# emiliofidalgo/liodom

Measured on AMD Instinct MI355X. Metric: scans/sec (64×1800 cloud, prev_frames=20) at 1 GPU; pose RMSE vs CPU ref, higher is better.
Workload: dtype f64

## Files before the change

### liodom_amd/csrc/handle_plan.h

```cpp
#pragma once
#include <algorithm>
#include <climits>
#include <cstdio>
#include <cstdlib>
#include <cstring>

#include "../../include/liodom_hip.h"
#include "liodom_sizes.h"

namespace liodom_dev {

struct HandleEnv {
  bool pipe_flags = true;
  bool map_rows = true;
  int hash_build = -1;
  int lds_cells_max = kLdsCellsMax;
  bool early_rebuild = true;
  bool safe_mode = false;
  int debug_clocks = 0;
  bool ring_split = true;
  bool ring_split_lb = true;
  int ring_pitch = 0;
  bool hash_incr = true;
  float rebuild_delta = 0.25f;
// ... 219 lines not shown
  const long long ring_pitch = env.ring_pitch ? env.ring_pitch : round_up(cdiv((long long)config->max_points * 9, (long long)H * 8), 8);

  if (ts > (1LL << 30) || map_cap > INT_MAX || used_cap > INT_MAX || sorted_cap > INT_MAX || ring_id_stride > INT_MAX || ring_pitch > INT_MAX) {
    *error = "liodom_create: capacities (window, received map, points per scan) exceed 32-bit sizes";
    return LIODOM_ERR_CAPACITY;
  }
  p.map_cap = (int)map_cap; p.table_size = (int)ts;
  p.used_cap = (int)used_cap; p.ovf_base = (int)ovf_base; p.sorted_cap = (int)sorted_cap;
  p.ring_id_stride = (size_t)ring_id_stride;
  p.ring_pitch = (int)ring_pitch;
  p.ring_stride = p.ring_split_lb ? std::max((size_t)config->max_points, (size_t)H * (size_t)p.ring_pitch) : (size_t)config->max_points;

  p.ring_split = env.ring_split && !p.safe_mode;
  if (p.ring_split) {
    long long budget = (long long)std::max(0, caps.ring_split_wgs_per_cu) * std::max(0, caps.cus) / 2;
    if (budget > 256) budget = 256;
    p.ring_split_max_wgs = (int)budget;
    if (p.tile_cap > p.ring_split_max_wgs) p.ring_split = false;
  }

  p.knn8 = p.lockstep && env.knn8;
  p.knn8_grid = (int)std::max(1LL, cdiv(cdiv(p.edge_cap, kKnn8Queries), kKnnGridDiv));
  p.hash_incr = (env.hash_incr && p.knn8 && p.lds_hash_build && !params->mapping && !params->filter_local_map && P > kHbPeriod &&
                 sorted_cap >= 2 * map_cap + (long long)(kHbPeriod - 1) * p.edge_cap) ? 1 : 0;
  p.hb_spill_base = p.sorted_cap - (kHbPeriod - 1) * p.edge_cap;
  p.knn_queries = p.lockstep ? 4 : 8;
  p.knn_partials = p.lockstep ? 0 : 1;
  p.knn_blocks = (int)round_up(cdiv(p.edge_cap, p.knn_queries), 4);
  p.knn_grid = (int)std::max(1LL, cdiv(p.knn_blocks, kKnnGridDiv));
  p.mask_stride = (int)round_up(p.knn_blocks, 128);

  p.ov_ok = env.knn_overlap != 0 && p.early_rebuild && S == 1 && p.knn_partials &&
            (env.knn_overlap == 2 || (long long)p.knn_grid * 4 * 3 <= (long long)caps.cus * 24);
  p.chain_ok = p.early_rebuild && S == 1 && p.knn_partials && !p.use_imu && (long long)p.knn_grid * 4 * 2 <= (long long)caps.cus * 24 &&
               env.knn_overlap != 0 && env.chain;
  p.speculate = (p.ov_ok || p.chain_ok) ? env.speculate : 0;
  p.spec_backoff = 16;
  p.spec_theta = env.spec_theta;

  *out = p;
  return LIODOM_OK;
}

struct OverlapModes { bool ov, chain; };
inline OverlapModes plan_overlap_modes(const HandlePlan& p, bool alone) {
  const bool base = p.early_rebuild && p.use_flags && alone;
  return {base && p.ov_ok, base && p.chain_ok && !p.flag_gate};
}

struct ModesRuntime {
  bool alone = true;
  bool streams_concurrent = true;
  int hb_stats[4] = {0, 0, 0, 0}, spec_stats[4] = {0, 0, 0, 0};
  unsigned int chain_count = 0, done0 = 0, done1 = 0;
  double replay_enqueue_us = 0.0, replay_wait_us = 0.0;
  int n_lagged = 0, n_readers = 0, n_hits = 0;
  long long subset_steps = 0;
};

inline void plan_format_modes(const HandlePlan& p, const ModesRuntime& r, char* buf, int cap) {
  const OverlapModes om = plan_overlap_modes(p, r.alone);
  snprintf(buf, (size_t)cap,
           "n_streams=%d early_rebuild=%d hash_build=%s pipe_flags=%d flag_gate=%d lm_groups=%d knn_instance=%d knn_queries=%d "
           "knn_grid=%d/%d knn8=%d hash_incr=%d hash_rebuilds=%d hash_appends=%d hash_appends_spilled=%d hash_points_spilled=%d knn_partials=%d knn_saved_bound=%d knn_exact_only=%d line_gate_kernel=%d filter_local_map=%d mapping=%d "
           "rotation_mode=%d table_size=%d sorted_cap=%d hb_spill_base=%d rebuild_delta=%.3f knn_overlap=%d streams_concurrent=%d safe_mode=%d ring_split=%d ring_split_max_wgs=%d ring_split_lb=%d chain=%d speculate=%d spec_early=%d/%d spec_unconfirmed=%d/%d chain_done=%u/%u/%u replay_enqueue_us=%.2f replay_wait_us=%.2f debug=%d",
           p.n_streams, p.early_rebuild, p.early_rebuild ? "streamed" : (p.lds_hash_build ? "lds" : "global"), p.use_flags ? 1 : 0,
           (p.use_flags && p.flag_gate) ? 1 : 0, p.lm_groups, p.lockstep ? 128 : 256, p.knn_queries, p.knn_grid,
           p.knn_blocks, p.knn8 ? 1 : 0, p.hash_incr, r.hb_stats[0], r.hb_stats[1], r.hb_stats[2], r.hb_stats[3], p.knn_partials,
           p.knn_save >= 2 ? 2 : (p.knn_save >= 1 ? 1 : 0), p.knn_exact_only, p.lockstep ? 1 : 0, p.filter_local_map, p.mapping,
           p.rotation_mode, p.table_size, p.sorted_cap, p.hb_spill_base, (double)p.rebuild_delta,
           (om.ov || om.chain) ? 1 : 0, r.streams_concurrent ? 1 : 0, p.safe_mode ? 1 : 0, p.ring_split ? 1 : 0, p.ring_split ? p.ring_split_max_wgs : 0, p.ring_split_lb ? 1 : 0,
           om.chain ? 1 : 0, p.speculate, r.spec_stats[0], r.spec_stats[2], r.spec_stats[1], r.spec_stats[3], r.chain_count, r.done0, r.done1,
           r.replay_enqueue_us, r.replay_wait_us, p.debug);
  auto tail = [&](size_t* room) { const size_t n = std::strlen(buf); *room = (size_t)cap - n; return buf + n; };
  size_t room = 0;
  if (p.pose_covariance) { char* t = tail(&room); snprintf(t, room, " pose_cov=1"); }
  if (r.n_lagged > 0) { char* t = tail(&room); snprintf(t, room, " mapper_lag=%d", r.n_lagged); }
  if (r.n_readers > 0) { char* t = tail(&room); snprintf(t, room, " map_readers=%d map_rows=%d", r.n_readers, p.map_rows ? 1 : 0); }
  if (r.n_hits > 0) { char* t = tail(&room); snprintf(t, room, " map_hits=%d", r.n_hits); }
  { char* t = tail(&room); snprintf(t, room, " subset_steps=%lld", r.subset_steps); }
}

}
```

### liodom_amd/csrc/kernels_knn.h

```cpp
constexpr float kCellInv = 1.0f;
constexpr double kCellSize = 1.0;

struct Top5 {
  unsigned long long k0, k1, k2, k3, k4;
  int p0, p1, p2, p3, p4;
};
constexpr unsigned long long kTop5Empty = (0x7f800000ull << 32) | 0x7fffffffull;
__device__ __forceinline__ float top5_dist(unsigned long long k) { return __int_as_float((int)(k >> 32)); }
__device__ __forceinline__ int top5_index(unsigned long long k) { return (int)(unsigned int)(k & 0xFFFFFFFFull); }
#define TOP5_STAGE(K, P)                                          \
  {                                                               \
    const bool lt = ck < (K);                                     \
    const unsigned long long nk = lt ? ck : (K);                  \
    const int np = lt ? cp : (P);                                 \
    ck = lt ? (K) : ck;                                           \
    cp = lt ? (P) : cp;                                           \
    (K) = nk; (P) = np;                                           \
  }
__device__ __forceinline__ void top5_insert(Top5& t, float d, int wi, int pos) {
  unsigned long long ck = ((unsigned long long)(unsigned int)__float_as_int(d) << 32) | (unsigned int)wi;
  int cp = pos;
  if (ck < t.k4) {
    TOP5_STAGE(t.k0, t.p0)
    TOP5_STAGE(t.k1, t.p1)
// ... 169 lines not shown


__device__ __forceinline__ void knn_merge(Top5& t, Top5& g, int hl, int half_shift) {
  unsigned long long gk[5]; int gp[5];
#pragma unroll
  for (int r = 0; r < 5; r++) {
    const unsigned long long key = t.k0;
    const unsigned int dmin = half_min_u32((unsigned int)(key >> 32));
    unsigned int win = (unsigned int)((__ballot((unsigned int)(key >> 32) == dmin) >> half_shift) & 0xFFFFFFFFull);
    unsigned long long mk;
    if (__popc(win) == 1) {
      mk = ((unsigned long long)dmin << 32) | (unsigned int)__shfl((int)(unsigned int)(key & 0xFFFFFFFFull), __ffs(win) - 1, kKnnGroup);
    } else {
      mk = half_min_u64(key);
      win = (unsigned int)((__ballot(key == mk) >> half_shift) & 0xFFFFFFFFull);
    }
    const int wl = __ffs(win) - 1;
    gp[r] = __shfl(t.p0, wl, kKnnGroup);
    gk[r] = mk;
    if (hl == wl) {
      t.k0 = t.k1; t.k1 = t.k2; t.k2 = t.k3; t.k3 = t.k4; t.k4 = kTop5Empty;
      t.p0 = t.p1; t.p1 = t.p2; t.p2 = t.p3; t.p3 = t.p4; t.p4 = -1;
    }
  }
  g.k0 = gk[0]; g.k1 = gk[1]; g.k2 = gk[2]; g.k3 = gk[3]; g.k4 = gk[4];
  g.p0 = gp[0]; g.p1 = gp[1]; g.p2 = gp[2]; g.p3 = gp[3]; g.p4 = gp[4];
}

__device__ void rebuild_alloc(const DevView& v, int s, StreamState& st, int block, int nblocks);
__device__ void rebuild_count_and_pad(const DevView& v, int s, StreamState& st, int eb, int block, int* sbase, int* sslot, bool keep);

template <int kQ>
struct KnnShared {
  int incl[kQ][kKnnGroup];
  int adj[kQ][kKnnGroup];
  float nn[kQ][16];
  int res[kQ][4];
  double part[kQ][32];
  double blk[kQ][24];
};

__device__ __forceinline__ float best2_bound(const Best2Acc& t, int half_shift) {
  float B = 1.0f;
  const float thr[4] = {0.36f, 0.09f, 0.0225f, 0.0036f};
#pragma unroll
  for (int k = 0; k < 4; k++) {
    const int c = __popc((unsigned int)(__ballot(t.m1 <= thr[k]) >> half_shift)) + __popc((unsigned int)(__ballot(t.m2 <= thr[k]) >> half_shift));
    B = c >= 5 ? thr[k] : B;
  }
  return B;
}

template <class Tune>
__device__ __forceinline__ void knn_probe_cells(const DevView& v, const StreamState& st, int fc, int hl, int cx, int cy, int cz, float qx, float qy, float qz,
                                                const CellSlot* cells, const unsigned int* bits, unsigned int tmask,
                                                unsigned int& start, unsigned int& cnt, float& lb) {
  if (hl < 27) {
    const int dx = hl % 3 - 1, dy = (hl / 3) % 3 - 1, dz = hl / 9 - 1;
    const unsigned long long key = pack_cell(cx + dx, cy + dy, cz + dz);
    unsigned int h = hash_cell(key, tmask);
    if (Tune::kProbeBoth) {
      const unsigned int word = bits[h >> 5];
      const uint4 raw = *reinterpret_cast<const uint4*>(cells + h);
      const unsigned long long k = ((unsigned long long)raw.y << 32) | raw.x;
      bool more = ((word >> (h & 31)) & 1u) != 0u;
      if (more && k == key) { start = raw.z; cnt = raw.w; more = false; }
      for (int pr = 1; more && pr < v.table_size; pr++) {
        h = (h + 1) & tmask;
        if (!((bits[h >> 5] >> (h & 31)) & 1u)) break;
        const uint4 r2 = *reinterpret_cast<const uint4*>(cells + h);
        if ((((unsigned long long)r2.y << 32) | r2.x) == key) { start = r2.z; cnt = r2.w; break; }
      }
    } else {
      for (int pr = 0; pr < v.table_size; pr++) {
        if (!((bits[h >> 5] >> (h & 31)) & 1u)) break;
        const uint4 raw = *reinterpret_cast<const uint4*>(cells + h);
        const unsigned long long k = ((unsigned long long)raw.y << 32) | raw.x;
        if (k == key) { start = raw.z; cnt = raw.w; break; }
        h = (h + 1) & tmask;
      }
    }
    const float cs = (float)kCellSize;
    const float lx = (float)(cx + dx) * cs, ly = (float)(cy + dy) * cs, lz = (float)(cz + dz) * cs;
    const float ex = qx < lx ? lx - qx : (qx > lx + cs ? qx - (lx + cs) : 0.0f);
    const float ey = qy < ly ? ly - qy : (qy > ly + cs ? qy - (ly + cs) : 0.0f);
    const float ez = qz < lz ? lz - qz : (qz > lz + cs ? qz - (lz + cs) : 0.0f);
    lb = (ex * ex + ey * ey + ez * ez) * (1.0f - 1e-5f);
  } else if (hl == 27 && v.early_rebuild) {
    start = (unsigned int)v.ovf_base;
    cnt = (unsigned int)st.n_ovf[LD_TAB_PARITY(v, fc)];
  }
}

struct KnnPre {
  float gsq;
  float4 sq;
  int p[5];
  float4 c[5];
};
constexpr float kOvMargin = 0.03f;
#ifndef LIODOM_OV_MARGIN_PER_M
#define LIODOM_OV_MARGIN_PER_M 0.004f
#endif
constexpr float kOvMarginPerMetre = LIODOM_OV_MARGIN_PER_M;
constexpr float kOvMarginMax = 0.30f;
template <int kKnnThreads>
__device__ __forceinline__ void knn_presearch(const DevView& v, int s, const StreamState& st, int fc, int e, int E,
                                              KnnShared<kKnnThreads / kKnnGroup>& sh, KnnPre& pre, float range) {
  typedef KnnTune<(kKnnThreads >= 256)> Tune;
  const int grp = threadIdx.x / kKnnGroup, hl = threadIdx.x & (kKnnGroup - 1);
  const int ec = e < v.edge_cap ? e : v.edge_cap - 1;
  pre.gsq = 0.f;
  pre.sq = make_float4(0.f, 0.f, 0.f, __int_as_float(0x7f800000));
#pragma unroll
  for (int k = 0; k < 5; k++) { pre.p[k] = -1; pre.c[k] = make_float4(0.f, 0.f, 0.f, 0.f); }
  if (!v.knn_save_q) return;
  pre.sq = v.knn_save_q[(size_t)s * v.edge_cap + ec];
  const float qx = pre.sq.x, qy = pre.sq.y, qz = pre.sq.z;
  const bool act = e < E && !v.knn_exact_only && ld_isfinite((double)qx) && ld_isfinite((double)qy) && ld_isfinite((double)qz) &&
                   fabsf(qx) < 1.0e9f && fabsf(qy) < 1.0e9f && fabsf(qz) < 1.0e9f;
  if (!act) return;
  const int cx = (int)floorf(qx * kCellInv), cy = (int)floorf(qy * kCellInv), cz = (int)floorf(qz * kCellInv);
  const unsigned int tmask = st.table_mask;
  const int stab = s + LD_TAB_PARITY(v, fc) * v.n_streams;
  const CellSlot* cells = v.cells + (size_t)stab * v.table_size;
  const unsigned int* bits = v.cell_bits + (size_t)stab * (v.table_size >> 5);
  const float4* sp = v.sorted_pts + (size_t)stab * v.sorted_cap;
  unsigned int start = 0, cnt = 0;
  float lb = 0.0f;
  knn_probe_cells<Tune>(v, st, fc, hl, cx, cy, cz, qx, qy, qz, cells, bits, tmask, start, cnt, lb);
  const float margin = fminf(kOvMargin + kOvMarginPerMetre * range, kOvMarginMax);
  const float r = fminf(sqrtf(pre.sq.w), 1.0f) + margin;
  const float B = r * r * (1.0f + 1e-5f);
  Top5Acc ta;
  {
    const unsigned long long sentinel = ((unsigned long long)(unsigned int)__float_as_int(B) << 32) | 0x7fffffffull;
    ta.t.k0 = ta.t.k1 = ta.t.k2 = ta.t.k3 = ta.t.k4 = sentinel;
    ta.t.p0 = ta.t.p1 = ta.t.p2 = ta.t.p3 = ta.t.p4 = -1;
  }
  const bool all = cnt > 0 && !(lb > B);
  knn_stream_cells<Top5Acc, 2, 2, 64>(ta, sp, sh.incl[grp], sh.adj[grp], start, all ? cnt : 0u, hl, qx, qy, qz);
  float gl = B;
  if (ta.t.p4 >= 0) gl = fminf(gl, top5_dist(ta.t.k4));
  pre.gsq = __int_as_float((int)half_min_u32((unsigned int)__float_as_int(gl)));
  pre.p[0] = ta.t.p0; pre.p[1] = ta.t.p1; pre.p[2] = ta.t.p2; pre.p[3] = ta.t.p3; pre.p[4] = ta.t.p4;
#pragma unroll
  for (int k = 0; k < 5; k++) pre.c[k] = sp[pre.p[k] >= 0 ? pre.p[k] : 0];
}

template <int kKnnThreads, bool kPre = false, bool kTail = true, bool kWt = kPre>
__device__ __forceinline__ void knn_block(const DevView& v, int s, StreamState& st, int fc, int outer_it, int eb, int bv, int E,
                                          KnnShared<kKnnThreads / kKnnGroup>& sh, const float4& p_in, const double (&T_in)[12],
                                          const KnnPre& pre, const double* qt) {
  constexpr int kKnnQueries = kKnnThreads / kKnnGroup;
  typedef KnnTune<(kKnnThreads >= 256)> Tune;
  const int grp = threadIdx.x / kKnnGroup;
  const int e = bv * kKnnQueries + grp;
  const int hl = threadIdx.x & (kKnnGroup - 1);
  const int half_shift = (threadIdx.x & 32);
  const bool dbgb = (bv == 5) && (s == 0) && (threadIdx.x == 0) && (outer_it == 0);
  const unsigned long long t_blk = (kInstrument && (v.debug & 32)) ? wall_clock64() : 0ull;
  DBG_STAMP(v, dbgb, 1, 0);
  bool active = e < E;
  float qx = 0.f, qy = 0.f, qz = 0.f;
  if (active) {
    float4 p = p_in;
    double T[12];
#pragma unroll
    for (int i = 0; i < 12; i++) T[i] = T_in[i];
    if (!Tune::kHoistLoads) {
      p = v.edges[((size_t)eb * v.n_streams + s) * v.edge_cap + e];
#pragma unroll
      for (int i = 0; i < 12; i++) T[i] = st.odom[i];
    }
    transform_point(T, p.x, p.y, p.z, &qx, &qy, &qz);
    if (v.knn_q && hl == 0) v.knn_q[((size_t)s * 2 + outer_it) * v.edge_cap + e] = make_float4(qx, qy, qz, 0.f);
    active = ld_isfinite((double)qx) && ld_isfinite((double)qy) && ld_isfinite((double)qz) &&
             fabsf(qx) < 1.0e9f && fabsf(qy) < 1.0e9f && fabsf(qz) < 1.0e9f;
  }
  DBG_STAMP(v, dbgb, 1, 1); DBG_QSTAMP(1);
  if (hl == 0) { sh.res[grp][0] = 0; sh.res[grp][1] = -1; sh.res[grp][2] = -1; }
  float d5 = __int_as_float(0x7f800000);
  if (active) {
    const int cx = (int)floorf(qx * kCellInv), cy = (int)floorf(qy * kCellInv), cz = (int)floorf(qz * kCellInv);
    const unsigned int tmask = st.table_mask;
    const int stab = s + LD_TAB_PARITY(v, fc) * v.n_streams;
    const CellSlot* cells = v.cells + (size_t)stab * v.table_size;
    const unsigned int* bits = v.cell_bits + (size_t)stab * (v.table_size >> 5);
    const float4* sp = v.sorted_pts + (size_t)stab * v.sorted_cap;
    float d5_r = __int_as_float(0x7f800000);
    int pos5[5] = {-1, -1, -1, -1, -1};
    bool reranked = false;
    if (kPre) {
      if ((kInstrument && (v.debug & 64)) && hl == 0 && !(pre.gsq > 0.f)) atomicAdd(&v.dbg_clk[262], 1ull);
      if (pre.gsq > 0.f) {
        Top5 t, g;
        top5_clear(t);
#pragma unroll
        for (int k = 0; k < 5; k++) {
          if (pre.p[k] >= 0) top5_insert(t, sqdist_f(qx, qy, qz, pre.c[k].x, pre.c[k].y, pre.c[k].z), __float_as_int(pre.c[k].w), pre.p[k]);
        }
        knn_merge(t, g, hl, half_shift);
        const float d5n = g.p4 >= 0 ? top5_dist(g.k4) : __int_as_float(0x7f800000);
        const double ddx = (double)qx - (double)pre.sq.x, ddy = (double)qy - (double)pre.sq.y, ddz = (double)qz - (double)pre.sq.z;
        const double delta = sqrt(ddx * ddx + ddy * ddy + ddz * ddz) * (1.0 + 1e-12);
        const double r = sqrt((double)pre.gsq) * (1.0 - 2e-7) - delta;
        double limit = r > 0.0 ? r * r * (1.0 - 1e-6) : 0.0;
        {
          const double cs = kCellSize;
          const double fx = (double)qx - (double)(int)floorf(pre.sq.x * kCellInv) * cs, fy = (double)qy - (double)(int)floorf(pre.sq.y * kCellInv) * cs,
                       fz = (double)qz - (double)(int)floorf(pre.sq.z * kCellInv) * cs;
          const double edge = fmin(fmin(fmin(fx, cs - fx), fmin(fy, cs - fy)), fmin(fz, cs - fz));
          const double ro = (cs + edge) * (1.0 - 2e-7);
          const double lo = ro > 0.0 ? ro * ro * (1.0 - 1e-6) : 0.0;
          limit = limit < lo ? limit : lo;
        }
        reranked = (double)d5n < limit || limit > 1.0;
        if ((kInstrument && (v.debug & 64)) && hl == 0) {
          atomicAdd(&v.dbg_clk[261], 1ull);
          if (!reranked) {
            const float rn = fminf(sqrtf(pre.sq.w), 1.0f) + kOvMargin;
            atomicAdd(&v.dbg_clk[g.p4 < 0 ? 264 : 265], 1ull);
            if (delta > 0.01) atomicAdd(&v.dbg_clk[266], 1ull);
            if (pre.gsq < rn * rn) atomicAdd(&v.dbg_clk[267], 1ull);
            if (!(pre.sq.w < 1.0f)) atomicAdd(&v.dbg_clk[268], 1ull);
            if (delta > 0.03) atomicAdd(&v.dbg_clk[269], 1ull);
          }
        }
        if (reranked) {
          d5_r = d5n;
          pos5[0] = g.p0; pos5[1] = g.p1; pos5[2] = g.p2; pos5[3] = g.p3; pos5[4] = g.p4;
          if (d5n < 1.0f) {
#pragma unroll
            for (int k = 0; k < 5; k++) {
              if (pre.p[k] >= 0) {
                const int r = pre.p[k] == g.p0 ? 0 : pre.p[k] == g.p1 ? 1 : pre.p[k] == g.p2 ? 2 : pre.p[k] == g.p3 ? 3 : pre.p[k] == g.p4 ? 4 : -1;
                if (r >= 0) {
                  sh.nn[grp][r * 3 + 0] = pre.c[k].x; sh.nn[grp][r * 3 + 1] = pre.c[k].y; sh.nn[grp][r * 3 + 2] = pre.c[k].z;
                  if (r < 2) sh.res[grp][1 + r] = __float_as_int(pre.c[k].w);
                }
              }
            }
            if (hl == 0) sh.res[grp][0] = 1;
          }
        }
      }
    } else
    if (outer_it == 1 && v.knn_save_pos && !v.knn_exact_only) {
      const float gsq = v.knn_save_g[(size_t)s * v.edge_cap + e];
      if (gsq > 0.f) {
        const float4 sq = v.knn_save_q[(size_t)s * v.edge_cap + e];
        const int2 sv = v.knn_save_pos[((size_t)s * v.edge_cap + e) * kKnnGroup + hl];
        const float4 m0 = sp[sv.x >= 0 ? sv.x : 0], m1 = sp[sv.y >= 0 ? sv.y : 0];
        Best2Acc br;
        br.clear();
        br.consider(sv.x >= 0, sqdist_f(qx, qy, qz, m0.x, m0.y, m0.z), 0, sv.x);
        br.consider(sv.y >= 0, sqdist_f(qx, qy, qz, m1.x, m1.y, m1.z), 0, sv.y);
        float d5n;
        int p5[5];
        const bool sel_ok = best2_select(br, hl, half_shift, d5n, p5);
        const double ddx = (double)qx - (double)sq.x, ddy = (double)qy - (double)sq.y, ddz = (double)qz - (double)sq.z;
        const double delta = sqrt(ddx * ddx + ddy * ddy + ddz * ddz) * (1.0 + 1e-12);
        const double r = sqrt((double)gsq) * (1.0 - 2e-7) - delta;
        const double limit = r > 0.0 ? r * r * (1.0 - 1e-6) : 0.0;
        reranked = sel_ok && ((double)d5n < limit || limit > 1.0);
        if (reranked) {
          d5_r = d5n;
#pragma unroll
          for (int k = 0; k < 5; k++) pos5[k] = p5[k];
        }
      }
    }
    if ((kInstrument && (v.debug & 64)) && hl == 0 && outer_it == 1) atomicAdd(&v.dbg_clk[259 + (reranked ? 0 : 1)], 1ull);
    if (!reranked) {
    unsigned int start = 0, cnt = 0;
    float lb = 0.0f;
    knn_probe_cells<Tune>(v, st, fc, hl, cx, cy, cz, qx, qy, qz, cells, bits, tmask, start, cnt, lb);
    DBG_STAMP(v, dbgb, 1, 2); DBG_QSTAMP(2);
    float B = 1.0f;
    bool have_b = false;
    if (outer_it == 1 && v.knn_save_q) {
      const float4 sq = kPre ? pre.sq : v.knn_save_q[(size_t)s * v.edge_cap + e];
      if (sq.w < 1.0f) {
        const float ddx = qx - sq.x, ddy = qy - sq.y, ddz = qz - sq.z;
        const float delta = sqrtf(ddx * ddx + ddy * ddy + ddz * ddz);
        const float r = sqrtf(sq.w) * (1.0f + 1e-6f) + delta * (1.0f + 1e-6f) + 1e-7f;
        B = fminf(1.0f, r * r * (1.0f + 1e-5f));
        have_b = true;
      }
    }
    bool pend = cnt > 0;
    Best2Acc b2;
    b2.clear();
    int dbg_n = 0;
    bool dbg_two_phase = false;
    {
      const bool now = pend && (have_b ? !(lb > B) : (hl == 13 || hl == 27 || lb <= Tune::kNearSq));
      if (kInstrument && (v.debug & 32)) dbg_n = __shfl(half_incl_scan_i32(now ? (int)cnt : 0), kKnnGroup - 1, kKnnGroup);
      knn_stream_cells<Best2Acc, Tune::kLoadsBig, Tune::kLoadsFlat, Tune::kBigCell, Tune::kCursor>(b2, sp, sh.incl[grp], sh.adj[grp], start, now ? cnt : 0u, hl, qx, qy, qz,
                                                                                     ((kInstrument && (v.debug & 32)) && s == 0 && e < E) ? v.dbg_q + ((size_t)outer_it * v.edge_cap + e) * 12 + 8 : nullptr);
      pend = pend && !now;
    }
    DBG_STAMP(v, dbgb, 1, 3); DBG_QSTAMP(3);
    if (!have_b && ((__ballot(pend) >> half_shift) & 0xFFFFFFFFull)) {
      B = best2_bound(b2, half_shift);
      pend = pend && !(lb > B);
      if ((__ballot(pend) >> half_shift) & 0xFFFFFFFFull) {
        if (kInstrument && (v.debug & 32)) { dbg_n += __shfl(half_incl_scan_i32(pend ? (int)cnt : 0), kKnnGroup - 1, kKnnGroup); dbg_two_phase = true; }
        knn_stream_cells<Best2Acc, Tune::kLoadsBig, Tune::kLoadsFlat, Tune::kBigCell, Tune::kCursor>(b2, sp, sh.incl[grp], sh.adj[grp], start, pend ? cnt : 0u, hl, qx, qy, qz);
      }
    } else {
      pend = false;
    }
    DBG_STAMP(v, dbgb, 1, 4); DBG_QSTAMP(4);
    const bool certain = best2_select(b2, hl, half_shift, d5, pos5) && !v.knn_exact_only;
    if ((kInstrument && (v.debug & 32)) && s == 0 && e < E && hl == 0) v.dbg_q[((size_t)outer_it * v.edge_cap + e) * 12] = (unsigned int)dbg_n | (dbg_two_phase ? 0x40000000u : 0u) | (certain ? 0u : 0x80000000u);
    if ((kInstrument && (v.debug & 64)) && hl == 0) {
      atomicAdd(&v.dbg_clk[256 + (certain ? 0 : 1)], 1ull);
      if (dbg_two_phase) atomicAdd(&v.dbg_clk[258], 1ull);
      atomicAdd(&v.dbg_clk[384 + (dbg_n / 64 < 63 ? dbg_n / 64 : 63)], 1ull);
    }
    if (!certain) {
      const bool all = cnt > 0 && (!(lb > B) || (!have_b && (hl == 13 || hl == 27 || lb <= Tune::kNearSq)));
      Top5Acc ta;
      Top5 g;
      {
        const float bnd = d5 < 1.0f ? d5 : 1.0f;
// ... 233 lines not shown
  static_assert(!(kOv && kChain), "the overlapped pass is the second pass, the chain-mode instance the first");
  StreamState& st = v.state[s];
  if (kOv) {
    if (!pipe_wait(v.ov_flags + s, seq, &st.status)) return false;
    OV_STAMP(v, threadIdx.x == 0 && bxi == 0, 9); OV_STAMP(v, threadIdx.x == 0 && bxi == v.knn_grid - 1, 13);
  } else if (kChain) {
    const bool pred_ok = pred_wait(v, s, bxi % kOvReplicas, (unsigned int)scan_no, sh_ov, &st.status, v.pipe_flags + eb, wait_edges, pred_copy);
    OV_STAMP(v, threadIdx.x == 0 && bxi == 0, 27);
    if (bxi == 0 && threadIdx.x == 0) { st.reb_frame_count = scan_no; st.n_used_tab[(scan_no + 1) & 1] = 0; st.reb_initialized = 1; st.cursor = 0; }
    if (pred_ok && bxi == 0 && threadIdx.x >= 64 && threadIdx.x < 76) st.pred_odom[scan_no & 1][threadIdx.x - 64] = sh_ov[threadIdx.x - 64];
    if (!pred_ok) return false;
  } else if (v.early_rebuild) {
    if (bxi >= v.knn_grid) { if (outer_it == 1) rebuild_alloc(v, s, st, bxi - v.knn_grid, (int)gridDim.x - v.knn_grid); return true; }
    if (outer_it == 0 && bxi == 0 && threadIdx.x == 0) {
      st.reb_frame_count = st.frame_count; st.n_used_tab[(st.frame_count + 1) & 1] = 0; st.reb_initialized = st.initialized;
      st.cursor = 0;
    }
    if (outer_it == 0 && bxi == 0 && threadIdx.x >= 64 && threadIdx.x < 76) st.pred_odom[st.frame_count & 1][threadIdx.x - 64] = st.odom[threadIdx.x - 64];
  }
  if (!kOv && outer_it == 0) {
    if (!kChain && signal_odo && bxi == 0 && byi == 0 && threadIdx.x == 0) {
      typedef __attribute__((address_space(1))) unsigned int gu32;
      __hip_atomic_store((gu32*)(v.pipe_flags + kEdgePipeBufs), signal_odo, __ATOMIC_RELAXED, __HIP_MEMORY_SCOPE_AGENT);
    }
    if (!kChain && wait_edges && !pipe_wait(v.pipe_flags + eb, wait_edges, &st.status)) return false;
  }
  typedef KnnTune<(kKnnThreads >= 256)> Tune;
  const int e_first = bxi * kKnnQueries + (int)(threadIdx.x / kKnnGroup);
  float4 p_first = make_float4(0.f, 0.f, 0.f, 0.f);
  double T[12] = {0, 0, 0, 0, 0, 0, 0, 0, 0, 0, 0, 0};
  if (Tune::kHoistLoads) {
    p_first = v.edges[((size_t)eb * v.n_streams + s) * v.edge_cap + (e_first < v.edge_cap ? e_first : v.edge_cap - 1)];
    if (!kOv && !kChain) {
#pragma unroll
      for (int i = 0; i < 12; i++) T[i] = st.odom[i];
    }
  }
  if (kChain) {
#pragma unroll
    for (int i = 0; i < 12; i++) T[i] = sh_ov[i];
  }
  const unsigned int st_status = st.status;
  const int st_init = kChain ? 1 : st.initialized;
  const int fc = kChain ? scan_no : st.frame_count;
  int E;
  if (kChain) {
    typedef __attribute__((address_space(1))) unsigned int gu32;
    E = (int)__hip_atomic_load((gu32*)(v.edge_cnt + eb * 32 + s), __ATOMIC_RELAXED, __HIP_MEMORY_SCOPE_AGENT);
  } else {
    E = st.n_edges_buf[eb];
  }
  if (st_status & LIODOM_STATUS_PIPE_TIMEOUT) return false;
  if (!st_init) return true;
  static_assert(kKnnGridDiv == 2, "k_knn handles exactly two query blocks per workgroup");
  constexpr bool kWt = kOv || kChain;
  if (bxi * kKnnQueries >= E) {
    if (threadIdx.x == 0) {
      unsigned char* cm = &v.corr_mask[((size_t)s * 2 + outer_it) * v.mask_stride + bxi];
      if (kWt) wt_store_u8(cm, 0); else *cm = 0;
      if (bxi + v.knn_grid < v.knn_blocks) { if (kWt) wt_store_u8(cm + v.knn_grid, 0); else cm[v.knn_grid] = 0; }
    }
    return true;
  }
  const int bv2 = bxi + v.knn_grid;
  const int e_second = bv2 * kKnnQueries + (int)(threadIdx.x / kKnnGroup);
  const bool second = bv2 < v.knn_blocks && bv2 * kKnnQueries < E;
  KnnPre pre1, pre2;
  float4 p_second = make_float4(0.f, 0.f, 0.f, 0.f);
  if (kOv) {
    if (second) p_second = v.edges[((size_t)eb * v.n_streams + s) * v.edge_cap + (e_second < v.edge_cap ? e_second : v.edge_cap - 1)];
    knn_presearch<kKnnThreads>(v, s, st, fc, e_first, E, sh, pre1, sqrtf(p_first.x * p_first.x + p_first.y * p_first.y + p_first.z * p_first.z));
    if (second) knn_presearch<kKnnThreads>(v, s, st, fc, e_second, E, sh2, pre2, sqrtf(p_second.x * p_second.x + p_second.y * p_second.y + p_second.z * p_second.z));
    else pre2.gsq = 0.f;
    if (!ov_wait_pose(v, s, bxi % kOvReplicas, seq, sh_ov, &st.status)) return false;
    OV_STAMP(v, threadIdx.x == 0 && bxi == 0, 10); OV_STAMP(v, threadIdx.x == 0 && bxi == v.knn_grid - 1, 14);
    if (kInstrument && (v.debug & 128) && threadIdx.x == 0) {
      sh_ov[19] = __longlong_as_double((long long)wall_clock64());
      const unsigned long long pub = *(volatile unsigned long long*)&v.dbg_clk[448 + 1];
      const long long d = (long long)wall_clock64() - (long long)pub;
      if (pub && d >= 0) atomicAdd(&v.dbg_clk[320 + (d / 25 < 63 ? d / 25 : 63)], 1ull);
    }
#pragma unroll
    for (int i = 0; i < 12; i++) T[i] = sh_ov[i];
  }
  if constexpr (kOv) {
    knn_block<kKnnThreads, true, false>(v, s, st, fc, outer_it, eb, bxi, E, sh, p_first, T, pre1, sh_ov + 12);
    if (second) knn_block<kKnnThreads, true, false>(v, s, st, fc, outer_it, eb, bv2, E, sh2, p_second, T, pre2, sh_ov + 12);
    else if (bv2 < v.knn_blocks && threadIdx.x == 0) wt_store_u8(&v.corr_mask[((size_t)s * 2 + outer_it) * v.mask_stride + bv2], 0);
    __syncthreads();
    knn_tail_dual<kKnnThreads>(v, s, outer_it, eb, bxi, bv2, second, E, sh, sh2, sh_ov + 12);
    if (!v.speculate) return true;
    const int cf = ov_confirm_pose(v, s, bxi % kOvReplicas, seq, sh_ov, &st.status);
    if ((kInstrument && (v.debug & 64)) && threadIdx.x == 0) atomicAdd(&v.dbg_clk[271 + (cf == 1 ? 0 : 1)], 1ull);
    return cf == 1;
  }
  knn_block<kKnnThreads, false, true, kWt>(v, s, st, fc, outer_it, eb, bxi, E, sh, p_first, T, pre1, kChain ? sh_ov + 12 : nullptr);
  if (bv2 >= v.knn_blocks) return true;
  if (!second) {
    if (threadIdx.x == 0) { unsigned char* cm = &v.corr_mask[((size_t)s * 2 + outer_it) * v.mask_stride + bv2]; if (kWt) wt_store_u8(cm, 0); else *cm = 0; }
    return true;
  }
  __syncthreads();
  double T2[12] = {0, 0, 0, 0, 0, 0, 0, 0, 0, 0, 0, 0};
  if (Tune::kHoistLoads) {
    p_second = v.edges[((size_t)eb * v.n_streams + s) * v.edge_cap + (e_second < v.edge_cap ? e_second : v.edge_cap - 1)];
    asm volatile("" ::: "memory");
// ... 173 lines not shown
```

### liodom_amd/csrc/liodom_hip.hip

```cpp
#include <hip/hip_runtime.h>

#include <algorithm>
#include <cmath>
#include <cstdint>
#include <cstdio>
#include <cstdlib>
#include <cstring>
#include <limits>
#include <atomic>
#include <chrono>
#include <mutex>
#include <optional>
#include <string>
#include <vector>

#include "liodom_kernels.h"
#include "handle_plan.h"
#include "step_plan.h"
#include "edge_pipe.h"
#include "map_attach.h"

using namespace liodom_dev;

namespace {
// ... 1865 lines not shown
  HIP_TRY(hipStreamSynchronize(h->stream_x));
  HIP_TRY(sync_odometry(h));
  HIP_TRY(hipMemcpyToSymbol(HIP_SYMBOL(g_inject_seed), &seed, sizeof(seed)));
  return LIODOM_OK;
#else
  (void)h; (void)seed;
  g_last_error = "liodom_debug_set_inject_seed: the product library carries no delay injection; build a variant with -DLIODOM_INJECT_DELAY (tools/variant_build.sh)";
  return LIODOM_ERR_UNSUPPORTED;
#endif
}

int liodom_debug_replay_stamps(liodom_handle_t* h, double* out_us, int cap) {
  if (!h || !out_us || cap < 0) return LIODOM_ERR_INVALID_ARG;
  const int n = (int)std::min<size_t>(h->replay_stamps.size(), (size_t)cap);
  for (int i = 0; i < n; i++) out_us[i] = h->replay_stamps[(size_t)i];
  return n;
}
int liodom_debug_clocks(liodom_handle_t* h, unsigned long long* out512) {
  if (!h || !out512) return LIODOM_ERR_INVALID_ARG;
  if (!kInstrument) { g_last_error = "liodom_debug_clocks: the product library carries no instrumentation; build a variant with -DLIODOM_INSTRUMENT (tools/variant_build.sh)"; return LIODOM_ERR_UNSUPPORTED; }
  if (int rc = enter(h)) return rc;
  SideLocks lk(h, true, true);
  HIP_TRY(hipStreamSynchronize(h->stream_x));
  HIP_TRY(sync_odometry(h));
  HIP_TRY(hipMemcpy(out512, h->v.dbg_clk, sizeof(unsigned long long) * 512, hipMemcpyDeviceToHost));
  return LIODOM_OK;
}

int liodom_debug_knn_times(liodom_handle_t* h, unsigned int* out, int* cap) {
  if (!h || !cap) return LIODOM_ERR_INVALID_ARG;
  *cap = h->v.edge_cap;
  if (!out) return LIODOM_OK;
  if (!h->v.dbg_q) return LIODOM_ERR_UNSUPPORTED;
  if (int rc = enter(h)) return rc;
  SideLocks lk(h, true, true);
  HIP_TRY(hipStreamSynchronize(h->stream_x));
  HIP_TRY(sync_odometry(h));
  HIP_TRY(hipMemcpy(out, h->v.dbg_q, sizeof(unsigned int) * 2 * (size_t)h->v.edge_cap * 12, hipMemcpyDeviceToHost));
  return LIODOM_OK;
}

int liodom_get_modes(liodom_handle_t* h, char* buf, int cap) {
  if (!h || !buf || cap < 2) return LIODOM_ERR_INVALID_ARG;
  if (int rc = enter(h)) return rc;
  SideLocks lk(h, true, true);
  const DevView& v = h->v;
  ModesRuntime r;
  r.alone = g_live_handles.load() <= 1;
  r.streams_concurrent = h->streams_concurrent;
  unsigned int done_cnt[64] = {0};
  if (v.knn_done0) (void)hipMemcpy(done_cnt, v.knn_done0, sizeof(done_cnt), hipMemcpyDeviceToHost);
  (void)hipMemcpy(r.spec_stats, reinterpret_cast<const char*>(v.state) + offsetof(StreamState, spec_stats), sizeof(r.spec_stats), hipMemcpyDeviceToHost);
  (void)hipMemcpy(r.hb_stats, reinterpret_cast<const char*>(v.state) + offsetof(StreamState, hb_stats), sizeof(r.hb_stats), hipMemcpyDeviceToHost);
  r.chain_count = h->step.chain_count; r.done0 = done_cnt[0]; r.done1 = done_cnt[32];
  if (h->replay_timed) { r.replay_enqueue_us = h->replay_enq_ns / (1e3 * (double)h->replay_timed); r.replay_wait_us = h->replay_wait_ns / (1e3 * (double)h->replay_timed); }
  r.n_lagged = h->maps.n_lagged; r.n_readers = h->maps.n_readers; r.subset_steps = h->subset_steps; r.n_hits = h->maps.n_hits;
  plan_format_modes(h->plan, r, buf, cap);
  return LIODOM_OK;
}

int liodom_device_count(int* count) {
  if (!count) return LIODOM_ERR_INVALID_ARG;
  int n = 0;
  if (hipGetDeviceCount(&n) != hipSuccess) n = 0;
  *count = n;
  return LIODOM_OK;
}

int liodom_device_pci_bus_id(int device, char* bus_id, int cap) {
  if (!bus_id || cap < 16) return LIODOM_ERR_INVALID_ARG;
  HIP_TRY(hipDeviceGetPCIBusId(bus_id, cap, device));
  return LIODOM_OK;
}

int liodom_device_info(liodom_handle_t* h, char* name, int name_cap, int* compute_units) {
  if (!h) return LIODOM_ERR_INVALID_ARG;
  hipDeviceProp_t prop;
  HIP_TRY(hipGetDeviceProperties(&prop, h->config.device));
  if (name && name_cap > 0) {
    const char* nm = prop.name[0] ? prop.name : prop.gcnArchName;
    std::strncpy(name, nm, (size_t)name_cap - 1); name[name_cap - 1] = 0;
  }
  if (compute_units) *compute_units = prop.multiProcessorCount;
  return LIODOM_OK;
}

}

#include "liodom_places_host.h"
#include "liodom_graph_host.h"
```

### liodom_amd/csrc/liodom_kernels.h

```cpp
#pragma once
#include <hip/hip_runtime.h>

#include <cstddef>

#include "../../include/liodom_hip.h"
#include "liodom_math.h"
#include "liodom_sizes.h"
#include "stream_state_format.h"
#include "wave_ops.h"

namespace liodom_dev {

#ifndef LIODOM_CHAIN_PRIO
#define LIODOM_CHAIN_PRIO 2
#endif
constexpr int kWave = 64;
constexpr uint64_t kEmptyKey = 0xFFFFFFFFFFFFFFFFull;
constexpr int kLmEvalThreads = kLmThreads;
constexpr int kLmCtl = kLmThreads - 64;
constexpr int kKnnGroup = 32;
constexpr int kEdgeBufX = 3;
constexpr int kOvReplicas = 8;
constexpr int kOvGranules = 38;
constexpr int kPredGranules = 38;
constexpr int kStreamLists = 2 * kEdgePipeBufs;
constexpr int kStreamListBase = 64;
constexpr int kStreamListChunk = 256;

struct StreamState {
  double odom[12];
  double prev_odom[12];
  double final_odom[12];
  double param_q[4];
  double param_t[3];
  int32_t initialized;
  int32_t append_raw;
  int32_t frame_count;
  int32_t n_frames;
  int32_t n_edges_buf[4];
  int32_t reb_frame_count;
  int32_t n_map;
  int32_t n_used_tab[2];
  int32_t cursor;
  int32_t scan_counter;
  uint32_t status;
  int32_t n_search;
  uint32_t table_mask;
  int32_t n_filt;
  int32_t vox_used;
  int32_t vox_cursor;
  int32_t vox_minb[3];
  int32_t vox_divb[3];
  int32_t n_recv;
  int32_t n_ovf[2];
  int32_t reb_initialized;
  int32_t reb_pad;
  int32_t spec_eval[2];
  int32_t hb_main_fc;
  int32_t hb_main_old;
  int32_t hb_main_nf;
  int32_t hb_base[8];
  int32_t hb_shift;
  int32_t hb_cursor;
  int32_t hb_stats[4];
  int32_t hb_spill;
  int32_t spec_redo[2];
  int32_t spec_stats[4];
  double pred_odom[2][12];
  liodom_step_info_t info;
};

struct __attribute__((aligned(16))) CellSlot {
  unsigned long long key;
  unsigned int start;
  unsigned int cnt;
};

#define LD_TAB_PARITY(v, frame_count) ((v).early_rebuild ? ((frame_count) & 1) : 0)

struct HostOut {
  double pose[7];
  liodom_step_info_t info;
  int seq;
  int pad;
};

struct PoseCovRaw {
  int scan_index, n_res, termination, has_solve;
  double cost;
  double H[21];
};
struct HostCov {
  liodom_pose_cov_t rec;
  int seq;
  int pad;
};

struct DevView {
  double min_range, max_range;
  int lidar_type, scan_lines, scan_regions, edges_per_region;
  long long min_points_per_scan;
  int prev_frames;
  int apply_on_ftol;
  int rotation_mode;
  int filter_local_map;
  int lm_groups;
  float vox_inv;
  int n_streams, max_points, ring_cap, slots_per_ring, edge_cap, map_cap, table_size;
  int pose_log_cap;
  int debug;
  StreamState* state;
  unsigned char* ring_id;   size_t ring_id_stride;
  unsigned short* tile_hist;
  int tile_cap;
  float4* ring_pts;
  int* ring_src;
  int* ring_start;
  int* ring_len;
  float4* edges_pad;
  int2* edges_pad_meta;
// ... 190 lines not shown
```

Measured before the change: 15070.

## Widen KNN presearch to a second cell shell so post-pose searches drop cell-face limits

Factors the hash-cell lookup and cell lower-bound into helpers. In the presearch it also scans one extra cell two steps out along the axis nearest the query, so the gathered ball covers a wider radius. The post-pose limit can then rely on ball distance alone and skip the cell-face clamp, which should let more queries reuse the presearch result instead of running a full search. It also adds always-on atomic counters for post-pose searches and total queries, which cost extra atomics per step, and the presearch now does more probing per query.

```diff
diff --git a/liodom_amd/csrc/handle_plan.h b/liodom_amd/csrc/handle_plan.h
--- a/liodom_amd/csrc/handle_plan.h
+++ b/liodom_amd/csrc/handle_plan.h
@@ -295,6 +295,7 @@
   bool alone = true;
   bool streams_concurrent = true;
   int hb_stats[4] = {0, 0, 0, 0}, spec_stats[4] = {0, 0, 0, 0};
+  int knn1_stats[2] = {0, 0};
   unsigned int chain_count = 0, done0 = 0, done1 = 0;
   double replay_enqueue_us = 0.0, replay_wait_us = 0.0;
   int n_lagged = 0, n_readers = 0, n_hits = 0;
@@ -322,6 +323,7 @@
   if (r.n_readers > 0) { char* t = tail(&room); snprintf(t, room, " map_readers=%d map_rows=%d", r.n_readers, p.map_rows ? 1 : 0); }
   if (r.n_hits > 0) { char* t = tail(&room); snprintf(t, room, " map_hits=%d", r.n_hits); }
   { char* t = tail(&room); snprintf(t, room, " subset_steps=%lld", r.subset_steps); }
-}
-
-}
+  if (r.knn1_stats[1] > 0) { char* t = tail(&room); snprintf(t, room, " knn1_post_pose_searches=%d knn1_queries=%d", r.knn1_stats[0], r.knn1_stats[1]); }
+}
+
+}
diff --git a/liodom_amd/csrc/kernels_knn.h b/liodom_amd/csrc/kernels_knn.h
--- a/liodom_amd/csrc/kernels_knn.h
+++ b/liodom_amd/csrc/kernels_knn.h
@@ -245,40 +245,49 @@
 }
 
 template <class Tune>
+__device__ __forceinline__ void knn_lookup_cell(const DevView& v, int ccx, int ccy, int ccz, const CellSlot* cells, const unsigned int* bits,
+                                                unsigned int tmask, unsigned int& start, unsigned int& cnt) {
+  const unsigned long long key = pack_cell(ccx, ccy, ccz);
+  unsigned int h = hash_cell(key, tmask);
+  if (Tune::kProbeBoth) {
+    const unsigned int word = bits[h >> 5];
+    const uint4 raw = *reinterpret_cast<const uint4*>(cells + h);
+    const unsigned long long k = ((unsigned long long)raw.y << 32) | raw.x;
+    bool more = ((word >> (h & 31)) & 1u) != 0u;
+    if (more && k == key) { start = raw.z; cnt = raw.w; more = false; }
+    for (int pr = 1; more && pr < v.table_size; pr++) {
+      h = (h + 1) & tmask;
+      if (!((bits[h >> 5] >> (h & 31)) & 1u)) break;
+      const uint4 r2 = *reinterpret_cast<const uint4*>(cells + h);
+      if ((((unsigned long long)r2.y << 32) | r2.x) == key) { start = r2.z; cnt = r2.w; break; }
+    }
+  } else {
+    for (int pr = 0; pr < v.table_size; pr++) {
+      if (!((bits[h >> 5] >> (h & 31)) & 1u)) break;
+      const uint4 raw = *reinterpret_cast<const uint4*>(cells + h);
+      const unsigned long long k = ((unsigned long long)raw.y << 32) | raw.x;
+      if (k == key) { start = raw.z; cnt = raw.w; break; }
+      h = (h + 1) & tmask;
+    }
+  }
+}
+__device__ __forceinline__ float knn_cell_lb(int ccx, int ccy, int ccz, float qx, float qy, float qz) {
+  const float cs = (float)kCellSize;
+  const float lx = (float)ccx * cs, ly = (float)ccy * cs, lz = (float)ccz * cs;
+  const float ex = qx < lx ? lx - qx : (qx > lx + cs ? qx - (lx + cs) : 0.0f);
+  const float ey = qy < ly ? ly - qy : (qy > ly + cs ? qy - (ly + cs) : 0.0f);
+  const float ez = qz < lz ? lz - qz : (qz > lz + cs ? qz - (lz + cs) : 0.0f);
+  return (ex * ex + ey * ey + ez * ez) * (1.0f - 1e-5f);
+}
+
+template <class Tune>
 __device__ __forceinline__ void knn_probe_cells(const DevView& v, const StreamState& st, int fc, int hl, int cx, int cy, int cz, float qx, float qy, float qz,
                                                 const CellSlot* cells, const unsigned int* bits, unsigned int tmask,
                                                 unsigned int& start, unsigned int& cnt, float& lb) {
   if (hl < 27) {
     const int dx = hl % 3 - 1, dy = (hl / 3) % 3 - 1, dz = hl / 9 - 1;
-    const unsigned long long key = pack_cell(cx + dx, cy + dy, cz + dz);
-    unsigned int h = hash_cell(key, tmask);
-    if (Tune::kProbeBoth) {
-      const unsigned int word = bits[h >> 5];
-      const uint4 raw = *reinterpret_cast<const uint4*>(cells + h);
-      const unsigned long long k = ((unsigned long long)raw.y << 32) | raw.x;
-      bool more = ((word >> (h & 31)) & 1u) != 0u;
-      if (more && k == key) { start = raw.z; cnt = raw.w; more = false; }
-      for (int pr = 1; more && pr < v.table_size; pr++) {
-        h = (h + 1) & tmask;
-        if (!((bits[h >> 5] >> (h & 31)) & 1u)) break;
-        const uint4 r2 = *reinterpret_cast<const uint4*>(cells + h);
-        if ((((unsigned long long)r2.y << 32) | r2.x) == key) { start = r2.z; cnt = r2.w; break; }
-      }
-    } else {
-      for (int pr = 0; pr < v.table_size; pr++) {
-        if (!((bits[h >> 5] >> (h & 31)) & 1u)) break;
-        const uint4 raw = *reinterpret_cast<const uint4*>(cells + h);
-        const unsigned long long k = ((unsigned long long)raw.y << 32) | raw.x;
-        if (k == key) { start = raw.z; cnt = raw.w; break; }
-        h = (h + 1) & tmask;
-      }
-    }
-    const float cs = (float)kCellSize;
-    const float lx = (float)(cx + dx) * cs, ly = (float)(cy + dy) * cs, lz = (float)(cz + dz) * cs;
-    const float ex = qx < lx ? lx - qx : (qx > lx + cs ? qx - (lx + cs) : 0.0f);
-    const float ey = qy < ly ? ly - qy : (qy > ly + cs ? qy - (ly + cs) : 0.0f);
-    const float ez = qz < lz ? lz - qz : (qz > lz + cs ? qz - (lz + cs) : 0.0f);
-    lb = (ex * ex + ey * ey + ez * ez) * (1.0f - 1e-5f);
+    knn_lookup_cell<Tune>(v, cx + dx, cy + dy, cz + dz, cells, bits, tmask, start, cnt);
+    lb = knn_cell_lb(cx + dx, cy + dy, cz + dz, qx, qy, qz);
   } else if (hl == 27 && v.early_rebuild) {
     start = (unsigned int)v.ovf_base;
     cnt = (unsigned int)st.n_ovf[LD_TAB_PARITY(v, fc)];
@@ -297,6 +306,9 @@
 #endif
 constexpr float kOvMarginPerMetre = LIODOM_OV_MARGIN_PER_M;
 constexpr float kOvMarginMax = 0.30f;
+#ifndef LIODOM_OV_BALL
+#define LIODOM_OV_BALL 1
+#endif
 template <int kKnnThreads>
 __device__ __forceinline__ void knn_presearch(const DevView& v, int s, const StreamState& st, int fc, int e, int E,
                                               KnnShared<kKnnThreads / kKnnGroup>& sh, KnnPre& pre, float range) {
@@ -333,6 +345,27 @@
   }
   const bool all = cnt > 0 && !(lb > B);
   knn_stream_cells<Top5Acc, 2, 2, 64>(ta, sp, sh.incl[grp], sh.adj[grp], start, all ? cnt : 0u, hl, qx, qy, qz);
+#if LIODOM_OV_BALL
+  static_assert((1.0 + kOvMarginMax) * (1.0 + kOvMarginMax) * 1.0001 < 1.99, "cells two steps out along two axes must lie beyond every collection radius");
+  static_assert(kOvMarginMax < 0.49f && kCellSize == 1.0, "cells behind a farther face must lie beyond every collection radius (gate 1.0 = one cell)");
+  {
+    int ex = 0, ey = 0, ez = 0;
+    bool want = false;
+    if (hl < 27) {
+      const int ax = hl / 9, u = (hl % 9) / 3 - 1, w = hl % 3 - 1;
+      const float cs = (float)kCellSize;
+      const float fa = ax == 0 ? qx - (float)cx * cs : (ax == 1 ? qy - (float)cy * cs : qz - (float)cz * cs);
+      const int two = fa < 0.5f * cs ? -2 : 2;
+      ex = cx + (ax == 0 ? two : u); ey = cy + (ax == 1 ? two : (ax == 0 ? u : w)); ez = cz + (ax == 2 ? two : w);
+      want = !(knn_cell_lb(ex, ey, ez, qx, qy, qz) > B);
+    }
+    if ((__ballot(want) >> (threadIdx.x & 32)) & 0xFFFFFFFFull) {
+      unsigned int start2 = 0, cnt2 = 0;
+      if (want) knn_lookup_cell<Tune>(v, ex, ey, ez, cells, bits, tmask, start2, cnt2);
+      knn_stream_cells<Top5Acc, 2, 2, 64>(ta, sp, sh.incl[grp], sh.adj[grp], start2, cnt2, hl, qx, qy, qz);
+    }
+  }
+#endif
   float gl = B;
   if (ta.t.p4 >= 0) gl = fminf(gl, top5_dist(ta.t.k4));
   pre.gsq = __int_as_float((int)half_min_u32((unsigned int)__float_as_int(gl)));
@@ -399,7 +432,8 @@
         const double delta = sqrt(ddx * ddx + ddy * ddy + ddz * ddz) * (1.0 + 1e-12);
         const double r = sqrt((double)pre.gsq) * (1.0 - 2e-7) - delta;
         double limit = r > 0.0 ? r * r * (1.0 - 1e-6) : 0.0;
-        {
+        const double limit_ball = limit;
+        if (!LIODOM_OV_BALL) {
           const double cs = kCellSize;
           const double fx = (double)qx - (double)(int)floorf(pre.sq.x * kCellInv) * cs, fy = (double)qy - (double)(int)floorf(pre.sq.y * kCellInv) * cs,
                        fz = (double)qz - (double)(int)floorf(pre.sq.z * kCellInv) * cs;
@@ -412,12 +446,16 @@
         if ((kInstrument && (v.debug & 64)) && hl == 0) {
           atomicAdd(&v.dbg_clk[261], 1ull);
           if (!reranked) {
-            const float rn = fminf(sqrtf(pre.sq.w), 1.0f) + kOvMargin;
+            const float rc = fminf(sqrtf(pre.sq.w), 1.0f) + fminf(kOvMargin + kOvMarginPerMetre * sqrtf(p_in.x * p_in.x + p_in.y * p_in.y + p_in.z * p_in.z), kOvMarginMax);
+            const double rf = (double)rc * (1.0 - 2e-7) - delta;
+            const double limit_full = rf > 0.0 ? rf * rf * (1.0 - 1e-6) : 0.0;
+            const bool same_cell = floorf(qx * kCellInv) == floorf(pre.sq.x * kCellInv) && floorf(qy * kCellInv) == floorf(pre.sq.y * kCellInv) && floorf(qz * kCellInv) == floorf(pre.sq.z * kCellInv);
+            const int why = ((double)d5n < limit_ball || limit_ball > 1.0) ? 266 : (((double)d5n < limit_full || limit_full > 1.0) ? 267 : (!(d5n < 1.0f) ? 269 : 263));
+            atomicAdd(&v.dbg_clk[why], 1ull);
             atomicAdd(&v.dbg_clk[g.p4 < 0 ? 264 : 265], 1ull);
-            if (delta > 0.01) atomicAdd(&v.dbg_clk[266], 1ull);
-            if (pre.gsq < rn * rn) atomicAdd(&v.dbg_clk[267], 1ull);
             if (!(pre.sq.w < 1.0f)) atomicAdd(&v.dbg_clk[268], 1ull);
-            if (delta > 0.03) atomicAdd(&v.dbg_clk[269], 1ull);
+            if (same_cell) atomicAdd(&v.dbg_clk[275], 1ull);
+            if (pre.gsq < rc * rc) atomicAdd(&v.dbg_clk[276], 1ull);
           }
         }
         if (reranked) {
@@ -466,6 +504,7 @@
     }
     if ((kInstrument && (v.debug & 64)) && hl == 0 && outer_it == 1) atomicAdd(&v.dbg_clk[259 + (reranked ? 0 : 1)], 1ull);
     if (!reranked) {
+    if (kPre && hl == 0) atomicAdd(&st.knn1_stats[0], 1);
     unsigned int start = 0, cnt = 0;
     float lb = 0.0f;
     knn_probe_cells<Tune>(v, st, fc, hl, cx, cy, cz, qx, qy, qz, cells, bits, tmask, start, cnt, lb);
@@ -805,6 +844,7 @@
   }
   if (st_status & LIODOM_STATUS_PIPE_TIMEOUT) return false;
   if (!st_init) return true;
+  if (kOv && bxi == 0 && threadIdx.x == 0 && E > 0) atomicAdd(&st.knn1_stats[1], E);
   static_assert(kKnnGridDiv == 2, "k_knn handles exactly two query blocks per workgroup");
   constexpr bool kWt = kOv || kChain;
   if (bxi * kKnnQueries >= E) {
diff --git a/liodom_amd/csrc/liodom_hip.hip b/liodom_amd/csrc/liodom_hip.hip
--- a/liodom_amd/csrc/liodom_hip.hip
+++ b/liodom_amd/csrc/liodom_hip.hip
@@ -1941,6 +1941,7 @@
   if (v.knn_done0) (void)hipMemcpy(done_cnt, v.knn_done0, sizeof(done_cnt), hipMemcpyDeviceToHost);
   (void)hipMemcpy(r.spec_stats, reinterpret_cast<const char*>(v.state) + offsetof(StreamState, spec_stats), sizeof(r.spec_stats), hipMemcpyDeviceToHost);
   (void)hipMemcpy(r.hb_stats, reinterpret_cast<const char*>(v.state) + offsetof(StreamState, hb_stats), sizeof(r.hb_stats), hipMemcpyDeviceToHost);
+  (void)hipMemcpy(r.knn1_stats, reinterpret_cast<const char*>(v.state) + offsetof(StreamState, knn1_stats), sizeof(r.knn1_stats), hipMemcpyDeviceToHost);
   r.chain_count = h->step.chain_count; r.done0 = done_cnt[0]; r.done1 = done_cnt[32];
   if (h->replay_timed) { r.replay_enqueue_us = h->replay_enq_ns / (1e3 * (double)h->replay_timed); r.replay_wait_us = h->replay_wait_ns / (1e3 * (double)h->replay_timed); }
   r.n_lagged = h->maps.n_lagged; r.n_readers = h->maps.n_readers; r.subset_steps = h->subset_steps; r.n_hits = h->maps.n_hits;
diff --git a/liodom_amd/csrc/liodom_kernels.h b/liodom_amd/csrc/liodom_kernels.h
--- a/liodom_amd/csrc/liodom_kernels.h
+++ b/liodom_amd/csrc/liodom_kernels.h
@@ -66,6 +66,7 @@
   int32_t hb_spill;
   int32_t spec_redo[2];
   int32_t spec_stats[4];
+  int32_t knn1_stats[2];
   double pred_odom[2][12];
   liodom_step_info_t info;
 };
```

Measured after the change: 14780. 0.981x the previous value.
